# masnottuh/point-cloud-toolbox

Measured on AMD Instinct MI355X. Metric: points/sec curvature (1M-pt torus, k=50); HBM GB/s k-NN vs peak, higher is better.
Workload: dtype f64

## Files before the change

point-cloud-toolbox_amd/csrc/pct_knn.hip:

```cpp
#include "pct_knn_sweep.h"

namespace {

__global__ __launch_bounds__(256) void k_plain_records(const float* __restrict__ xyz, int64_t n, float4* __restrict__ out) {
    const int64_t i = (int64_t)blockIdx.x * 256 + threadIdx.x;
    if (i < n) out[i] = make_float4(xyz[3 * i], xyz[3 * i + 1], xyz[3 * i + 2], __int_as_float((int)i));
}

template <int R>
__global__ __launch_bounds__(64 * kWavesPerBlock) void k_query_points(const float4* __restrict__ pts, int n, const double* __restrict__ q_xyz,
                                                                      int64_t m, int k, double eps2, int* __restrict__ idx_out,
                                                                      double* __restrict__ dist_out) {
    __shared__ double s_pend_d[kWavesPerBlock][64 * R + 64];
    __shared__ int s_pend_p[kWavesPerBlock][64 * R + 64];
    const int w = __builtin_amdgcn_readfirstlane(threadIdx.x >> 6);
    const int lane = lane_id();
    const int64_t q = (int64_t)blockIdx.x * kWavesPerBlock + w;
    if (q >= m) return;
    Sweep<R> sw;
    sw.k = k - 1;
    sw.eps2 = eps2;
    sw.pts = pts;
    sw.pend_d = s_pend_d[w];
    sw.pend_p = s_pend_p[w];
// ... 175 lines not shown
    ctx->tm.sweep_variant = p.variant();
    return PCT_OK;
}

}

int pct_launch_knn_grid(pct_ctx* ctx, int32_t k, double eps, bool exact_only, int phase, bool want_dist, pct_call_clock* clock) {
    const int64_t n_rows = ctx->own_flag ? ctx->own_count : ctx->q_end - ctx->q_begin;
    const SweepPlan plan = plan_for(ctx, k, eps, false, exact_only, phase, want_dist);
    if (phase != 2) {
        PCT_TRY(reserve_table(ctx, k, eps, plan.dist));
        PCT_TRY(pct_reserve(ctx, &ctx->redo, ((size_t)n_rows + 16) * sizeof(int)));
        if (ctx->level_mode) PCT_TRY(pct_reserve(ctx, &ctx->redo_m, ((size_t)n_rows + 16) * sizeof(int)));
    }
    KnnArgs a = make_args(ctx, k, eps, true);
    if (!ctx->dist_valid) a.nbr_dist = nullptr;
    int* redo_count = &pct_dev(ctx)->sweep.redo_count;
    int* redo = (int*)ctx->redo.p;
    const dim3 block(64 * kWavesPerBlock);
    const bool fast = plan.family != kNoSweep;
    a.stamp_sweep = clock->word(PCT_ST_GRID_END);
    a.stamp_exact = clock->word(fast ? PCT_ST_FAST_END : PCT_ST_GRID_END);
    a.stamp_exact_also = fast ? nullptr : clock->word(PCT_ST_FAST_END);
    PCT_TRY(launch_sweep(ctx, plan, a, redo, redo_count));
    PCT_HIP(ctx, clock->boundary(PCT_ST_FAST_END, ctx->stream));
    if (phase != 1) {
        const int64_t waves = exact_only ? n_rows : 32768;
        const int blocks = (int)((waves + kWavesPerBlock - 1) / kWavesPerBlock);
        const int* list = exact_only ? nullptr : redo;
        if (k + 1 <= 64)
            PCT_LAUNCH(k_knn_exact<1>, dim3(blocks), block, 0, ctx->stream, a, list, (const int*)redo_count);
        else if (k + 1 <= 128)
            PCT_LAUNCH(k_knn_exact<2>, dim3(blocks), block, 0, ctx->stream, a, list, (const int*)redo_count);
        else
            PCT_TRY(pct_launch_knn_exact_wide(ctx, a, blocks, list, (const int*)redo_count));
        PCT_HIP(ctx, hipGetLastError());
    }
    ctx->knn_sorted_space = true;
    return PCT_OK;
}

int pct_launch_knn_tree(pct_ctx* ctx, int32_t k, double eps, bool want_dist, pct_call_clock* clock) {
    if (ctx->level_mode || ctx->own_flag || ctx->q_begin != 0 || ctx->q_end != ctx->n)
        return pct_fail(ctx, PCT_ERR_INVALID, "the tree sweep takes whole clouds");
    const int64_t n_rows = ctx->n;
    const bool exact_only = pct_getenv("PCT_TREE_EXACT_ONLY") != nullptr;
// ... 122 lines not shown
```

point-cloud-toolbox_amd/csrc/pct_knn_duo.hip:

```cpp
#include "pct_knn_item.h"

namespace {

#include "pct_sort_duo.inc"

__device__ __forceinline__ void sort_duo_asm(unsigned& ea, unsigned& eb, const SortLanes& c) {
    unsigned ta, tb;
    asm volatile(PCT_SORT_DUO_ASM
                 : [ea] "+v"(ea), [eb] "+v"(eb), [ta] "=&v"(ta), [tb] "=&v"(tb)
                 : [sel0] "v"(c.sel[0]), [sel1] "v"(c.sel[1]), [sel2] "v"(c.sel[2]), [sel3] "v"(c.sel[3]), [sel4] "v"(c.sel[4]),
                   [sel5] "v"(c.sel[5]), [a31] "v"(c.a31), [a63] "v"(c.a63));
    const unsigned lo = PCT_SORT_DUO_RESULT_A, hi = PCT_SORT_DUO_RESULT_B;
    ea = lo;
    eb = hi;
}

#ifndef PCT_DUO_CAP
#define PCT_DUO_CAP 768
#endif
constexpr int kDuoCap = PCT_DUO_CAP;
template <bool DIST, int CAP>
struct DuoLds {
    float cx[CAP], cy[CAP], cz[CAP];
    unsigned short pend[128 + 8];
// ... 6 lines not shown
__global__ __launch_bounds__(64, ((TREE ? PCT_TREE_CAP2 : PCT_DUO_CAP) <= 768 ? 4 : 3)) void k_knn_duo(PairArgs a) {
    constexpr int CAP = TREE ? PCT_TREE_CAP2 : kDuoCap, LIST = 128, SLOT_BITS = 7, KEY_BITS = 32 - SLOT_BITS;
    static_assert(CAP % 128 == 0 && CAP <= 1024, "slot ids: 10 bits of slot, 4 bits of run index");
    __shared__ DuoLds<DIST, CAP> L;
    const int lane = lane_id();
    const int item = a.items_per_xcd ? ((int)blockIdx.x & 7) * a.items_per_xcd + ((int)blockIdx.x >> 3) : (int)blockIdx.x;
    if (item >= a.n_items) return;
    const SortLanes sort_dir = make_sort_lanes();
    constexpr int NRUNS = TREE ? 27 : 9;
    const int2 it2 = a.items[item];
    if (item_of_split_segment<TREE>(it2)) return;
    ItemHead<TREE> head;
    load_item_head<TREE>(a, it2, lane, head);
    const int cx = head.cx, cy = head.cy, cz = head.cz, qs = head.qs, nq = head.nq, row0 = head.row0;
    const int run_s = head.run_s, run_len = head.run_len;
    const pct_grid& G = TREE ? head.g_lvl : a.g;
    float4 my_q;
    double my_qx, my_qy, my_qz;
    float my_eq;
    load_queries<Q64>(a.pts, a.ptsd, qs, nq, lane, my_q, my_qx, my_qy, my_qz, my_eq);
    int my_pre, m;
    run_prefix<NRUNS>(run_len, lane, my_pre, m);
    pct_stamp(a.stamp);
    if (item_overflows<TREE, NRUNS>(m, CAP, run_len, lane)) {
        hand_item_to_redo(a.redo, a.redo_count, a.counters, a.stats, row0, nq, lane, true);
        return;
    }
    unsigned slotx[CAP / 64];
    {
        unsigned* bits = (unsigned*)L.pend;
        static_assert(sizeof(L.pend) >= CAP / 8, "the run-start bit string lives in the survivor list");
        if (lane < CAP / 32) bits[lane] = 0u;
        wave_lds_sync();
        const bool nonempty = lane < NRUNS && run_len > 0;
        const unsigned long long ne = __builtin_amdgcn_ballot_w64(nonempty);
        if (nonempty) {
            atomicOr(&bits[my_pre >> 5], 1u << (my_pre & 31));
            L.offc[__builtin_amdgcn_mbcnt_lo((unsigned)ne, 0)] = run_s - my_pre;
        }
        wave_lds_sync();
        float4 tmp[CAP / 64];
        int ubase = -1;
#pragma unroll
        for (int b = 0; b < CAP / 64; ++b) {
            tmp[b] = make_float4(0.f, 0.f, 0.f, 0.f);
            slotx[b] = (unsigned)(b * 64 + lane);
            if (b * 64 < m) {
                const unsigned lo = (unsigned)__builtin_amdgcn_readfirstlane((int)bits[2 * b]);
                const unsigned hi = (unsigned)__builtin_amdgcn_readfirstlane((int)bits[2 * b + 1]);
                const unsigned long long B = ((unsigned long long)hi << 32) | lo;
                const unsigned long long S = B >> 1;
                const int s0 = ubase + (int)(lo & 1u);
                const int u = (int)__builtin_amdgcn_mbcnt_hi((unsigned)(S >> 32), __builtin_amdgcn_mbcnt_lo((unsigned)S, (unsigned)s0));
                ubase += (int)__popcll(B);
                const int j = b * 64 + lane;
                slotx[b] |= (unsigned)u << 10;
                if (j < m) tmp[b] = a.pts[j + L.offc[u]];
// ... 3 lines not shown
#pragma unroll
        for (int b = 0; b < CAP / 64; ++b) {
            const int j = b * 64 + lane;
            if (j < m) {
                L.cx[j] = tmp[b].x; L.cy[j] = tmp[b].y; L.cz[j] = tmp[b].z;
            } else if ((b & ~1) * 64 < m) {
                L.cx[j] = INFINITY; L.cy[j] = 0.f; L.cz[j] = 0.f;
            }
        }
    }
    wave_lds_sync();

    const int k = a.k;
    const double eps2 = EPS ? a.eps2 : (double)INFINITY;
    const KeySetup<KEY_BITS> keys = make_key_setup<KEY_BITS, EPS>(G, cx, cy, cz, my_q, Q64, my_qx, my_qy, my_qz, eps2);
    const double scale = keys.scale;
    constexpr unsigned key_max = KeySetup<KEY_BITS>::key_max;
    const unsigned my_gkey = keys.my_gkey;
    const float cell2f = keys.cell2f;
    const unsigned eps_key = EPS ? keys.eps_key : 0xFFFFFFFFu;
    const float eps2a = EPS ? keys.eps2a : INFINITY;
    const double eps1 = EPS ? keys.eps1 : 0.0;
    float t_prev_f = 0.f;
    unsigned long long redo_mask = 0ull;

    char* const pos_item = (char*)(a.nbr_pos + (int64_t)row0 * a.pitch);
    char* const dist_item = DIST ? (char*)(a.nbr_dist + (int64_t)row0 * a.pitch) : nullptr;
    const unsigned pitch4 = (unsigned)a.pitch * 4u;
    const unsigned lane_off0 = (unsigned)(lane - 1) * 4u, lane_off1 = (unsigned)(lane + 63) * 4u;
    const bool col0 = lane >= 1 && lane <= k, col1 = lane + 64 <= k;
    const unsigned long long order_lo = k >= 63 ? ~0ull : (2ull << k) - 1ull;
    const unsigned long long order_hi = k < 64 ? 0ull : k - 64 >= 63 ? ~0ull : (2ull << (k - 64)) - 1ull;
    const unsigned short* pend_hi = &L.pend[64];

    const auto query_loop = [&](auto NBP_) {
        constexpr int NBP = decltype(NBP_)::value, NBU = 2 * NBP;
        for (int qi = 0; qi < nq; ++qi) {
            const float ax = __int_as_float(__builtin_amdgcn_readlane(__float_as_int(my_q.x), qi));
            const float ay = __int_as_float(__builtin_amdgcn_readlane(__float_as_int(my_q.y), qi));
            const float az = __int_as_float(__builtin_amdgcn_readlane(__float_as_int(my_q.z), qi));
            const auto rl64 = [&](double v, int l) {
                return __hiloint2double(__builtin_amdgcn_readlane(__double2hiint(v), l), __builtin_amdgcn_readlane(__double2loint(v), l));
            };
            const double qx = Q64 ? rl64(my_qx, qi) : (double)ax, qy = Q64 ? rl64(my_qy, qi) : (double)ay, qz = Q64 ? rl64(my_qz, qi) : (double)az;
            const float eq = Q64 ? __int_as_float(__builtin_amdgcn_readlane(__float_as_int(my_eq), qi)) : 0.f;
            float ap[NBU];
#pragma unroll
// ... 22 lines not shown
            float T = T_init;
            int cnt = tot;
            unsigned bkey = 0xFFFFFFFFu;
            if (need) {
                const float target = 0.5f * (float)(k + 1 + LIST);
                float t = t_prev_f > 0.f ? t_prev_f : cell2f;
                if (!(t < T_init)) t = 0.5f * T_init;
                float lo = 0.f, hi = T_init;
                bool found = false;
#pragma unroll 1
                for (int trial = 0; trial < 16; ++trial) {
                    int c = 0;
#pragma unroll
                    for (int b = 0; b < NBU; ++b) c += (int)__popcll(__builtin_amdgcn_ballot_w64(ap[b] < t));
                    if ((unsigned)(c - (k + 1)) <= (unsigned)(LIST - (k + 1))) { T = t; cnt = c; found = true; break; }
                    const bool below = c < k + 1;
                    lo = below ? t : lo;
                    hi = below ? hi : t;
                    float nt = t * target * __builtin_amdgcn_rcpf((float)c);
                    if (!(nt > lo && nt < hi)) nt = hi < INFINITY ? 0.5f * (lo + hi) : 2.f * lo;
                    if (__builtin_amdgcn_ballot_w64(!(nt > lo && nt < hi)) != 0ull) break;
                    t = nt;
                }
                if (!found || __builtin_amdgcn_ballot_w64(!(T >= 1e-30f)) != 0ull) { redo_mask |= 1ull << qi; continue; }
                t_prev_f = T;
                double lo2 = (double)T * (1.0 - 0x1p-20);
                if constexpr (Q64) {
                    const double root_up = (double)__builtin_sqrtf(T) * (1.0 + 0x1p-21);
                    lo2 = fmax(lo2 - 2.0 * (double)eq * root_up, 0.0);
                }
                bkey = (unsigned)fmin(lo2 * scale, 4294967294.0);
            }
            {
                unsigned wr = (unsigned)(uintptr_t)&L.pend[0], wr1;
                const unsigned long long all = __builtin_amdgcn_read_exec();
                wave_lds_sync();
#pragma unroll
                for (int b = 0; b < NBU; b += 2) {
                    unsigned r0, r1, n0, n1;
                    asm volatile(
                        "v_cmp_gt_f32 vcc, %[t], %[ap0]\n"
                        "v_cmp_gt_f32 s[96:97], %[t], %[ap1]\n"
                        "s_bcnt1_i32_b64 %[n0], vcc\n"
                        "v_mbcnt_lo_u32_b32 %[r0], vcc_lo, 0\n"
                        "s_bcnt1_i32_b64 %[n1], s[96:97]\n"
                        "v_mbcnt_lo_u32_b32 %[r1], s96, 0\n"
                        "v_mbcnt_hi_u32_b32 %[r0], vcc_hi, %[r0]\n"
                        "v_mbcnt_hi_u32_b32 %[r1], s97, %[r1]\n"
                        "s_lshl1_add_u32 %[wr1], %[n0], %[wr]\n"
                        "v_lshl_add_u32 %[r0], %[r0], 1, %[wr]\n"
                        "v_lshl_add_u32 %[r1], %[r1], 1, %[wr1]\n"
                        "s_mov_b64 exec, vcc\n"
                        "ds_write_b16 %[r0], %[slot0]\n"
                        "s_mov_b64 exec, s[96:97]\n"
// ... 11 lines not shown
            unsigned e[2];
            {
                const double dx0 = (double)L.cx[j0] - qx, dy0 = (double)L.cy[j0] - qy, dz0 = (double)L.cz[j0] - qz;
                const double dx1 = (double)L.cx[j1] - qx, dy1 = (double)L.cy[j1] - qy, dz1 = (double)L.cz[j1] - qz;
                const double d20 = (dx0 * dx0 + dy0 * dy0) + dz0 * dz0;
                const double d21 = (dx1 * dx1 + dy1 * dy1) + dz1 * dz1;
                L.pay_p[lane] = j0 + L.offc[sx0 >> 10];
                L.pay_p[lane + 64] = j1 + L.offc[sx1 >> 10];
                if constexpr (DIST) {
                    L.pay_d[lane] = (float)sqrt(d20);
                    L.pay_d[lane + 64] = (float)sqrt(d21);
                }
                const unsigned k0 = (min((unsigned)(d20 * scale), key_max - 1u) << SLOT_BITS) | (unsigned)lane;
                const unsigned k1 = (min((unsigned)(d21 * scale), key_max - 1u) << SLOT_BITS) | (unsigned)(lane + 64);
                e[0] = lane < cnt && (!EPS || d20 < eps2) ? k0 : kPadElem;
                e[1] = lane + 64 < cnt && (!EPS || d21 < eps2) ? k1 : kPadElem;
            }
            wave_lds_sync();
            sort_duo_asm(e[0], e[1], sort_dir);
            const unsigned tau = (unsigned)__builtin_amdgcn_readlane((int)(k < 64 ? e[0] : e[1]), k & 63);
            const unsigned gk = (unsigned)__builtin_amdgcn_readlane((int)my_gkey, qi);
            const unsigned tk = tau >> SLOT_BITS;
            const unsigned need_k = min(tau == kPadElem ? 0xFFFFFFFFu : tk + 1u, eps_key);
            if (need_k > min(gk, bkey) || (tau != kPadElem && tk >= key_max - 1u)) { redo_mask |= 1ull << qi; continue; }
            {
                unsigned n0, n1;
                asm("s_nop 1\n"
                    "v_mov_b32_dpp %0, %2 wave_shl:1 row_mask:0xf bank_mask:0xf bound_ctrl:1\n"
                    "v_mov_b32_dpp %1, %3 wave_shl:1 row_mask:0xf bank_mask:0xf bound_ctrl:1\n"
                    "s_nop 0"
                    : "=&v"(n0), "=&v"(n1) : "v"(e[0]), "v"(e[1]));
                n0 = lane == 63 ? (unsigned)__builtin_amdgcn_readlane((int)e[1], 0) : n0;
                const bool same0 = ((e[0] ^ n0) >> SLOT_BITS) == 0u && e[0] != kPadElem && n0 != kPadElem;
                const bool same1 = ((e[1] ^ n1) >> SLOT_BITS) == 0u && e[1] != kPadElem && n1 != kPadElem && lane < 63;
                const unsigned long long cm = (__builtin_amdgcn_ballot_w64(same0) & order_lo) | (__builtin_amdgcn_ballot_w64(same1) & order_hi);
                if (__builtin_expect(cm != 0ull, 0)) {
                    const bool done = order_equal_keys<2, SLOT_BITS>(e, a.pts,
                        [&](unsigned at) {
                            const int j = min((int)L.pend[at] & 1023, CAP - 1);
                            const double dx = (double)L.cx[j] - qx, dy = (double)L.cy[j] - qy, dz = (double)L.cz[j] - qz;
                            return (dx * dx + dy * dy) + dz * dz;
                        },
                        [&](unsigned at) { return L.pay_p[at]; });
                    if (!done) { redo_mask |= 1ull << qi; continue; }
                }
            }
            {
                const unsigned off0 = lane_off0 + (unsigned)qi * pitch4, off1 = lane_off1 + (unsigned)qi * pitch4;
                const bool real0 = e[0] != kPadElem, real1 = e[1] != kPadElem;
                const int s0 = (int)(e[0] & 127u), s1 = (int)(e[1] & 127u);
                const int pos0 = L.pay_p[s0], pos1 = L.pay_p[s1];
                if (col0) *(int*)(pos_item + off0) = real0 ? pos0 : -1;
                if (col1) *(int*)(pos_item + off1) = real1 ? pos1 : -1;
                if constexpr (DIST) {
                    const float d0 = L.pay_d[s0], d1 = L.pay_d[s1];
                    if (col0) *(float*)(dist_item + off0) = real0 ? d0 : INFINITY;
                    if (col1) *(float*)(dist_item + off1) = real1 ? d1 : INFINITY;
                }
                if constexpr (EPS) {
                    const int f = (int)__popcll(__builtin_amdgcn_ballot_w64(real0 && col0)) + (int)__popcll(__builtin_amdgcn_ballot_w64(real1 && col1));
                    if (lane == 0) a.nbr_cnt[row0 + qi] = f;
                }
            }
            wave_lds_sync();
        }
    };
    {
// ... 34 lines not shown
```

point-cloud-toolbox_amd/csrc/pct_knn_fast.hip:

```cpp
#include "pct_knn_item.h"

namespace {


#ifndef PCT_FAST_WAVES
#define PCT_FAST_WAVES 4
#endif
template <int R> constexpr int kFastWaves = PCT_FAST_WAVES;



template <int R, bool EPS, bool PRE, bool PAIR = false, bool Q64 = false, bool TREE = false>
__global__ __launch_bounds__(64 * kFastWaves<R>, (TREE ? (R == 1 ? (PCT_TREE_CAP <= 512 ? 6 : PCT_TREE_CAP <= 768 ? 4 : 3) : (PCT_TREE_CAP2 <= 768 ? 4 : 3)) : R == 1 ? (Q64 ? 5 : 6) : 4)) void k_knn_fast(KnnArgs a, const int2* __restrict__ items, int64_t n_items,
                                                                  int items_q, int* __restrict__ redo,
                                                                  int* __restrict__ redo_count) {
    constexpr int CAP = TREE ? (R == 1 ? PCT_TREE_CAP : PCT_TREE_CAP2) : R == 1 ? kStageCap : PCT_STAGE_CAP2;
    constexpr int SLOT_BITS = PRE ? (R == 1 ? 6 : 7) : (R == 1 ? 9 : 10);
    constexpr int KEY_BITS = 32 - SLOT_BITS;
    constexpr int CAP_POW2 = 1024;
    static_assert(CAP <= CAP_POW2, "staging capacity");
    static_assert(PRE || CAP <= (1 << SLOT_BITS), "slot field too narrow");
    __shared__ float s_cx[kFastWaves<R>][CAP];
    __shared__ float s_cy[kFastWaves<R>][CAP];
    __shared__ float s_cz[kFastWaves<R>][CAP];
// ... 68 lines not shown
    if constexpr (Q64) {
        const double ex = my_qd.x - (double)my_q.x, ey = my_qd.y - (double)my_q.y, ez = my_qd.z - (double)my_q.z;
        my_eq = (float)sqrt((ex * ex + ey * ey) + ez * ez) * (1.0f + 0x1p-22f);
        if (!(my_eq >= 0.f)) my_eq = INFINITY;
    }
    int my_pre, m;
    run_prefix<NRUNS>(run_len, lane, my_pre, m);
    pct_stamp(a.stamp_sweep);
    unsigned long long n_flush = 0, n_step = 0, n_redo = 0;
    unsigned long long redo_mask = 0ull, redo_why_lo = 0ull, redo_why_hi = 0ull;
    const auto note_redo = [&](int row, int why) {
        const int q = row - row0;
        redo_mask |= 1ull << q;
        redo_why_lo |= (unsigned long long)(why & 1) << q;
        redo_why_hi |= (unsigned long long)((why >> 1) & 1) << q;
    };

    const bool hopeless = !EPS && a.row_done != nullptr && m < a.k + 1;
    if (item_overflows<TREE, NRUNS>(m, CAP, run_len, lane) || hopeless) {
        if (a.row_done) {
            if (lane < nq) a.redo_m[row0 + lane] = ((hopeless ? 1 : 2) << 29) | min(m, (1 << 29) - 1);
            return;
        }
        hand_item_to_redo(redo, redo_count, a.counters, a.stats, row0, nq, lane, !hopeless);
        return;
    }

    unsigned run_code[(CAP / 64 + 7) / 8];
#pragma unroll
    for (int i = 0; i < (CAP / 64 + 7) / 8; ++i) run_code[i] = 0u;
    {
        unsigned* bits = pend;
        static_assert(CAP / 32 <= 64 * R, "bit string does not fit the list area");
        if (lane < CAP / 32) bits[lane] = 0u;
        wave_lds_sync();
        const bool nonempty = lane < NRUNS && run_len > 0;
        const unsigned long long ne = __builtin_amdgcn_ballot_w64(nonempty);
        if (nonempty) {
            atomicOr(&bits[my_pre >> 5], 1u << (my_pre & 31));
            offc[__builtin_amdgcn_mbcnt_lo((unsigned)ne, 0)] = run_s - my_pre;
        }
        wave_lds_sync();
        float4 tmp[CAP / 64];
        int ubase = -1;
#pragma unroll
        for (int b = 0; b < CAP / 64; ++b) {
            tmp[b] = make_float4(0.f, 0.f, 0.f, 0.f);
// ... 686 lines not shown
```

point-cloud-toolbox_amd/csrc/pct_knn_item.h:

```cpp
#pragma once
#include "pct_knn_net.h"

namespace {

typedef float float2v __attribute__((ext_vector_type(2)));

struct PairArgs {
    const float4* pts;
    const double4* ptsd;
    const int* cell_start;
    const int* cell_own;
    const int* own_start;
    const int2* items;
    int* nbr_pos;
    float* nbr_dist;
    int* nbr_cnt;
    int* redo;
    int* redo_count;
    pct_sweep_words* counters;
    int n_items, items_q;
    int items_per_xcd;
    int k, pitch;
    int stats;
    unsigned magic_x, magic_xy;
    int shift_x, shift_xy;
    double eps2;
    pct_grid g;
    const int4* tree_seg;
    const int2* tree_runs;
    int tree_bits;
    unsigned long long* stamp;
};

PairArgs make_pair_args(const pct_ctx* ctx, const KnnArgs& a, bool tree, int* redo, int* redo_count) {
    PairArgs pa = {};
    pa.pts = a.pts; pa.ptsd = a.ptsd; pa.cell_start = a.cell_start;
    pa.items = (const int2*)ctx->occ.p;
    pa.nbr_pos = a.nbr_pos; pa.nbr_dist = a.nbr_dist; pa.nbr_cnt = a.nbr_cnt;
    pa.redo = redo; pa.redo_count = redo_count; pa.counters = a.counters;
    pa.n_items = (int)ctx->n_items; pa.items_q = ctx->items_q;
    pa.k = a.k; pa.pitch = a.pitch; pa.stats = a.stats; pa.eps2 = a.eps2; pa.g = a.g;
    pa.stamp = a.stamp_sweep;
    pa.items_per_xcd = pct_getenv("PCT_NO_XCD_MAP") ? 0 : (int)((ctx->n_items + 7) / 8);
    if (tree) {
        pa.tree_seg = a.tree_seg; pa.tree_runs = a.tree_runs; pa.tree_bits = a.tree_bits;
        return pa;
    }
    pa.cell_own = a.cell_own; pa.own_start = a.own_start;
    const auto magic = [](unsigned d, unsigned* mg, int* sh) {
        int l = 0;
        while ((1ull << l) < d) ++l;
        *sh = 30 + l;
        *mg = (unsigned)(((1ull << *sh) + d - 1) / d);
    };
    magic((unsigned)a.g.nx, &pa.magic_x, &pa.shift_x);
    magic((unsigned)a.g.nx * (unsigned)a.g.ny, &pa.magic_xy, &pa.shift_xy);
    return pa;
}

template <class F, class... Rest>
void with_bools(F&& f, bool b, Rest... rest) {
    if constexpr (sizeof...(rest) == 0) {
        if (b) f(std::true_type{}); else f(std::false_type{});
    } else {
// ... 74 lines not shown
        }
    }
}

template <int NRUNS>
__device__ __forceinline__ void run_prefix(const int run_len, const int lane, int& my_pre, int& m) {
    my_pre = 0;
    int acc = 0;
#pragma unroll
    for (int t = 0; t < NRUNS; ++t) {
        my_pre = lane == t ? acc : my_pre;
        acc += __builtin_amdgcn_readlane(run_len, t);
    }
    m = acc;
}

template <bool TREE, int NRUNS>
__device__ __forceinline__ bool item_overflows(const int m, const int cap, const int run_len, const int lane) {
    const bool crowded = TREE && __popcll(__builtin_amdgcn_ballot_w64(lane < NRUNS && run_len > 0)) > 16;
    return m > cap || crowded;
}

__device__ __forceinline__ void hand_item_to_redo(int* __restrict__ redo, int* __restrict__ redo_count, pct_sweep_words* counters,
                                                  const int stats, const int row0, const int nq, const int lane, const bool overflow) {
    int base = 0;
    if (lane == 0) base = atomicAdd(redo_count, nq);
    base = __builtin_amdgcn_readfirstlane(base);
    if (lane < nq) redo[base + lane] = row0 + lane;
    if (stats && lane == 0) {
        if (overflow) atomicAdd(&counters->lds_overflows, 1ull);
        atomicAdd(&counters->redone_queries, (unsigned long long)nq);
    }
}

template <bool Q64>
__device__ __forceinline__ void load_queries(const float4* pts, const double4* ptsd, const int qs, const int nq,
                                             const int lane, float4& my_q, double& my_qx, double& my_qy, double& my_qz, float& my_eq) {
    my_q = make_float4(0.f, 0.f, 0.f, 0.f);
    my_qx = 0.; my_qy = 0.; my_qz = 0.;
    my_eq = 0.f;
    if (lane < nq) {
        my_q = pts[qs + lane];
        if constexpr (Q64) {
            const double4 qd = ptsd[qs + lane];
            my_qx = qd.x; my_qy = qd.y; my_qz = qd.z;
        }
    }
    if constexpr (Q64) {
        const double ex = my_qx - (double)my_q.x, ey = my_qy - (double)my_q.y, ez = my_qz - (double)my_q.z;
        my_eq = (float)sqrt((ex * ex + ey * ey) + ez * ez) * (1.0f + 0x1p-22f);
        if (!(my_eq >= 0.f)) my_eq = INFINITY;
// ... 38 lines not shown
```

point-cloud-toolbox_amd/csrc/pct_knn_pair.hip:

```cpp
#include "pct_knn_item.h"

namespace {

#ifndef PCT_SORT_INC
#define PCT_SORT_INC "pct_sort_pair.inc"
#endif
#include PCT_SORT_INC

__device__ __forceinline__ void sort_pair_asm(unsigned& ea, unsigned& eb, const SortLanes& c) {
    unsigned ta, tb;
    asm volatile(PCT_SORT_PAIR_ASM
                 : [ea] "+v"(ea), [eb] "+v"(eb), [ta] "=&v"(ta), [tb] "=&v"(tb)
                 : [sel0] "v"(c.sel[0]), [sel1] "v"(c.sel[1]), [sel2] "v"(c.sel[2]), [sel3] "v"(c.sel[3]), [sel4] "v"(c.sel[4]),
                   [sel5] "v"(c.sel[5]), [a31] "v"(c.a31), [a63] "v"(c.a63));
    ea = PCT_SORT_PAIR_RESULT_A;
    eb = PCT_SORT_PAIR_RESULT_B;
}

constexpr int kPairCap = kStageCap;
static_assert((kPairCap & (kPairCap - 1)) == 0 && kPairCap % 128 == 0 && kPairCap <= 512, "staging capacity of k_knn_pair");
static_assert(PCT_TREE_CAP % 128 == 0 && PCT_TREE_CAP <= 1024, "staging capacity of k_knn_pair on the hierarchical cell list");
template <int CAP>
struct PairLdsT {
    float cx[CAP], cy[CAP], cz[CAP];
// ... 16 lines not shown
    __shared__ PairLdsT<CAP> s_lds[kPairWaves];
    const int w = kPairWaves == 1 ? 0 : __builtin_amdgcn_readfirstlane(threadIdx.x >> 6);
    const int lane = lane_id();
    const int blk = (int)blockIdx.x * kPairWaves + w;
    const int item = a.items_per_xcd ? (blk & 7) * a.items_per_xcd + (blk >> 3) : blk;
    if (item >= a.n_items || (a.items_per_xcd && (blk >> 3) >= a.items_per_xcd)) return;
    PairLdsT<CAP>& L = s_lds[w];
    const SortLanes sort_dir = make_sort_lanes();
    constexpr int NRUNS = TREE ? 27 : 9;
    const int2 it2 = a.items[item];
    if (item_of_split_segment<TREE>(it2)) return;
    ItemHead<TREE> head;
    load_item_head<TREE>(a, it2, lane, head);
    const int cx = head.cx, cy = head.cy, cz = head.cz, qs = head.qs, nq = head.nq, row0 = head.row0;
    const int run_s = head.run_s, run_len = head.run_len;
    const pct_grid& G = TREE ? head.g_lvl : a.g;
    float4 my_q;
    double my_qx, my_qy, my_qz;
    float my_eq;
    load_queries<Q64>(a.pts, a.ptsd, qs, nq, lane, my_q, my_qx, my_qy, my_qz, my_eq);
    int my_pre, m;
    run_prefix<NRUNS>(run_len, lane, my_pre, m);
    pct_stamp(a.stamp);
    if (item_overflows<TREE, NRUNS>(m, CAP, run_len, lane)) {
        hand_item_to_redo(a.redo, a.redo_count, a.counters, a.stats, row0, nq, lane, true);
        return;
    }

    unsigned slotx[CAP / 64];
    {
        unsigned* bits = L.pend;
        if (lane < CAP / 32) bits[lane] = 0u;
        wave_lds_sync();
        const bool nonempty = lane < NRUNS && run_len > 0;
        const unsigned long long ne = __builtin_amdgcn_ballot_w64(nonempty);
        if (nonempty) {
            atomicOr(&bits[my_pre >> 5], 1u << (my_pre & 31));
            L.offc[__builtin_amdgcn_mbcnt_lo((unsigned)ne, 0)] = run_s - my_pre;
        }
        wave_lds_sync();
        float4 tmp[CAP / 64];
        int ubase = -1;
#pragma unroll
        for (int b = 0; b < CAP / 64; ++b) {
            tmp[b] = make_float4(0.f, 0.f, 0.f, 0.f);
            slotx[b] = (unsigned)(b * 64 + lane);
            if (b * 64 < m) {
                const unsigned lo = (unsigned)__builtin_amdgcn_readfirstlane((int)bits[2 * b]);
                const unsigned hi = (unsigned)__builtin_amdgcn_readfirstlane((int)bits[2 * b + 1]);
                const unsigned long long B = ((unsigned long long)hi << 32) | lo;
                const unsigned long long S = B >> 1;
                const int s0 = ubase + (int)(lo & 1u);
                const int u = (int)__builtin_amdgcn_mbcnt_hi((unsigned)(S >> 32), __builtin_amdgcn_mbcnt_lo((unsigned)S, (unsigned)s0));
                ubase += (int)__popcll(B);
                const int j = b * 64 + lane;
                slotx[b] |= (unsigned)u << SB;
                if (j < m) tmp[b] = a.pts[j + L.offc[u]];
// ... 3 lines not shown
#pragma unroll
        for (int b = 0; b < CAP / 64; ++b) {
            const int j = b * 64 + lane;
            if (j < m) {
                L.cx[j] = tmp[b].x; L.cy[j] = tmp[b].y; L.cz[j] = tmp[b].z;
            } else if ((b & ~1) * 64 < m) {
                L.cx[j] = INFINITY; L.cy[j] = 0.f; L.cz[j] = 0.f;
            }
        }
    }
    wave_lds_sync();

    const int k = a.k;
    const double eps2 = EPS ? a.eps2 : (double)INFINITY;
    const KeySetup<KEY_BITS> keys = make_key_setup<KEY_BITS, EPS>(G, cx, cy, cz, my_q, Q64, my_qx, my_qy, my_qz, eps2);
    const double scale = keys.scale;
    constexpr unsigned key_max = KeySetup<KEY_BITS>::key_max;
    const unsigned my_gkey = keys.my_gkey;
    const float cell2f = keys.cell2f;
    const unsigned eps_key = EPS ? keys.eps_key : 0xFFFFFFFFu;
    const float eps2a = EPS ? keys.eps2a : INFINITY;
    const double eps1 = EPS ? keys.eps1 : 0.0;
    float t_prev_f = 0.f;
    unsigned long long redo_mask = 0ull;

    char* const pos_item = (char*)(a.nbr_pos + (int64_t)row0 * a.pitch);
    char* const dist_item = DIST ? (char*)(a.nbr_dist + (int64_t)row0 * a.pitch) : nullptr;
    const unsigned lane_off = (unsigned)(lane - 1) * 4u;
    const unsigned pitch4 = (unsigned)a.pitch * 4u;
    const bool col_lane = lane >= 1 && lane <= k;
    const unsigned long long first_k1 = (2ull << k) - 1ull;

    static_assert(CAP <= (1 << SB) && SB + 4 <= 16, "slot ids: SB bits of slot, 4 bits of run index, 16-bit survivor list of query b");
    const auto slot_of = [](unsigned id) { return TREE ? min((int)(id & ((1u << SB) - 1u)), CAP - 1) : (int)(id & (unsigned)(CAP - 1)); };

    const auto pair_loop = [&](auto NBP_) {
        constexpr int NBP = decltype(NBP_)::value, NBU = 2 * NBP;
        for (int qi = 0; qi < nq; qi += 2) {
            const bool live_b = qi + 1 < nq;
            const int qj = live_b ? qi + 1 : qi;
            const float ax = __int_as_float(__builtin_amdgcn_readlane(__float_as_int(my_q.x), qi));
            const float ay = __int_as_float(__builtin_amdgcn_readlane(__float_as_int(my_q.y), qi));
            const float az = __int_as_float(__builtin_amdgcn_readlane(__float_as_int(my_q.z), qi));
            const float bx = __int_as_float(__builtin_amdgcn_readlane(__float_as_int(my_q.x), qj));
            const float by = __int_as_float(__builtin_amdgcn_readlane(__float_as_int(my_q.y), qj));
            const float bz = __int_as_float(__builtin_amdgcn_readlane(__float_as_int(my_q.z), qj));
            const auto rl64 = [&](double v, int l) {
// ... 83 lines not shown
                    float nt = v_t * target * __builtin_amdgcn_rcpf((float)c);
                    if (!(nt > v_lo && nt < v_hi)) nt = v_hi < INFINITY ? 0.5f * (v_lo + v_hi) : 2.f * v_lo;
                    go = go && nt > v_lo && nt < v_hi;
                    v_t = go ? nt : v_t;
                    if ((__builtin_amdgcn_ballot_w64(go) & 3ull) == 0ull) break;
                }
                const unsigned fm = (unsigned)__builtin_amdgcn_ballot_w64(found);
                T_a = __int_as_float(__builtin_amdgcn_readlane(__float_as_int(v_T), 0));
                T_b = __int_as_float(__builtin_amdgcn_readlane(__float_as_int(v_T), 1));
                cnt_a = __builtin_amdgcn_readlane(v_cnt, 0);
                cnt_b = __builtin_amdgcn_readlane(v_cnt, 1);
                double lo2 = (double)v_T * (1.0 - 0x1p-20);
                if constexpr (Q64) {
                    const double root_up = (double)__builtin_sqrtf(v_T) * (1.0 + 0x1p-21);
                    lo2 = fmax(lo2 - 2.0 * (double)v_eq * root_up, 0.0);
                }
                const unsigned v_bkey = (unsigned)fmin(lo2 * scale, 4294967294.0);
                ok_a = (fm & 1u) != 0u && (!need_a || T_a >= 1e-30f);
                ok_b = live_b && (fm & 2u) != 0u && (!need_b || T_b >= 1e-30f);
                if (need_a && ok_a) { t_prev_f = T_a; bkey_a = (unsigned)__builtin_amdgcn_readlane((int)v_bkey, 0); }
                if (need_b && ok_b) { t_prev_f = T_b; bkey_b = (unsigned)__builtin_amdgcn_readlane((int)v_bkey, 1); }
                if (!ok_a) { redo_mask |= 1ull << qi; T_a = 0.f; cnt_a = 0; }
                if (!ok_b) { if (live_b) redo_mask |= 1ull << qj; T_b = 0.f; cnt_b = 0; }
                if (!ok_a && !ok_b) continue;
            }
            if (!live_b) { T_b = 0.f; cnt_b = 0; }
            {
                unsigned wr_a = (unsigned)(uintptr_t)&L.pend[0], wr_b = (unsigned)(uintptr_t)&L.pend_b[0];
                const unsigned long long all = __builtin_amdgcn_read_exec();
                wave_lds_sync();
#ifndef PCT_ABL_NO_COMPACT
#pragma unroll
                for (int b = 0; b < NBU; ++b) {
                    unsigned ra, rb, ca, cb;
                    const unsigned slot = slotx[b];
                    asm volatile(
                        "v_cmp_gt_f32 vcc, %[ta], %[apa]\n"
                        "v_cmp_gt_f32 s[96:97], %[tb], %[apb]\n"
                        "s_bcnt1_i32_b64 %[ca], vcc\n"
                        "v_mbcnt_lo_u32_b32 %[ra], vcc_lo, 0\n"
                        "s_bcnt1_i32_b64 %[cb], s[96:97]\n"
                        "v_mbcnt_lo_u32_b32 %[rb], s96, 0\n"
                        "v_mbcnt_hi_u32_b32 %[ra], vcc_hi, %[ra]\n"
                        "v_mbcnt_hi_u32_b32 %[rb], s97, %[rb]\n"
                        "v_lshl_add_u32 %[ra], %[ra], 2, %[wra]\n"
                        "v_lshl_add_u32 %[rb], %[rb], 1, %[wrb]\n"
                        "s_mov_b64 exec, vcc\n"
// ... 84 lines not shown
                            [&](unsigned at) {
                                const int j = slot_of((unsigned)L.pend_b[at]);
                                const double dx = (double)L.cx[j] - ux, dy = (double)L.cy[j] - uy, dz = (double)L.cz[j] - uz;
                                return (dx * dx + dy * dy) + dz * dz;
                            },
                            [&](unsigned at) { return __builtin_amdgcn_ds_bpermute((int)(at & 63u) << 2, out_pb); });
                        if (!done) { redo_mask |= 1ull << qj; ok_b = false; }
                    }
                }
            }
            {
                const unsigned off_a = lane_off + (unsigned)qi * pitch4, off_b = lane_off + (unsigned)qj * pitch4;
                const bool real_a = e_a != kPadElem, real_b = e_b != kPadElem;
                const int at_a = (int)(e_a << 2), at_b = (int)(e_b << 2);
                const int pos_a = __builtin_amdgcn_ds_bpermute(at_a, out_pa), pos_b = __builtin_amdgcn_ds_bpermute(at_b, out_pb);
                float dist_a = 0.f, dist_b = 0.f;
                if constexpr (DIST) {
                    dist_a = __int_as_float(__builtin_amdgcn_ds_bpermute(at_a, __float_as_int(out_da)));
                    dist_b = __int_as_float(__builtin_amdgcn_ds_bpermute(at_b, __float_as_int(out_db)));
                }
#ifdef PCT_ABL_NO_STORE
                if (pos_a == 0x7fffffff && pos_b == 0x7ffffff1)
#endif
                if (ok_a && col_lane) {
                    *(int*)(pos_item + off_a) = real_a ? pos_a : -1;
                    if constexpr (DIST) *(float*)(dist_item + off_a) = real_a ? dist_a : INFINITY;
                }
#ifdef PCT_ABL_NO_STORE
                if (pos_a == 0x7fffffff && pos_b == 0x7ffffff1)
#endif
                if (ok_b && col_lane) {
                    *(int*)(pos_item + off_b) = real_b ? pos_b : -1;
                    if constexpr (DIST) *(float*)(dist_item + off_b) = real_b ? dist_b : INFINITY;
                }
                if constexpr (EPS) {
                    const int f_a = (int)__popcll(__builtin_amdgcn_ballot_w64(real_a && col_lane));
                    const int f_b = (int)__popcll(__builtin_amdgcn_ballot_w64(real_b && col_lane));
                    if (lane == 0) {
                        if (ok_a) a.nbr_cnt[row0 + qi] = f_a;
                        if (ok_b) a.nbr_cnt[row0 + qj] = f_b;
                    }
                }
            }
        }
    };
    {
        using std::integral_constant;
        const int nbp = (m + 127) >> 7;
        if (nbp <= 1) pair_loop(integral_constant<int, 1>{});
        else if (nbp == 2) pair_loop(integral_constant<int, 2>{});
        else if (nbp == 3) pair_loop(integral_constant<int, (CAP >= 384 ? 3 : 1)>{});
        else if (nbp == 4) pair_loop(integral_constant<int, (CAP >= 512 ? 4 : 1)>{});
        else if (nbp == 5) pair_loop(integral_constant<int, (CAP >= 640 ? 5 : 1)>{});
        else pair_loop(integral_constant<int, (CAP >= 768 ? 6 : 1)>{});
// ... 28 lines not shown
```

point-cloud-toolbox_amd/csrc/pct_knn_sweep.h:

```cpp
#pragma once
#include "pct_internal.h"
#include "pct_query_plan.h"
#include "pct_sweep_plan.h"

#include <math.h>
#include <type_traits>

struct KnnArgs {
    const float4* pts;
    const double4* ptsd;
    const int* cell_start;
    const int* cell_own;
    const int* own_start;
    const int* owned_pos;
    int64_t n_owned;
    const int* occ;
    int64_t n_occ;
    int64_t n;
    pct_grid g;
    int k;
    int pitch;
    double eps2;
    int q_begin, q_end;
    int* nbr_pos;
    float* nbr_dist;
    int* nbr_cnt;
    int* row_done;
    int* redo_m;
    const int4* tree_seg;
    const int2* tree_runs;
    int tree_bits;
    const unsigned long long* tree_codes;
    const unsigned char* tree_lvl;
    const int* tree_bucket;
    int stats;
    pct_sweep_words* counters;
    unsigned long long* stamp_sweep;
    unsigned long long* stamp_exact;
    unsigned long long* stamp_exact_also;
};

int pct_launch_knn_exact_wide(pct_ctx* ctx, const KnnArgs& a, int blocks, const int* list, const int* list_count);
int pct_launch_knn_brute_wide(pct_ctx* ctx, const KnnArgs& a, int blocks);
void pct_launch_sweep_fast(pct_ctx* ctx, const SweepPlan& p, const KnnArgs& a, int* redo, int* redo_count);
void pct_launch_sweep_pair(pct_ctx* ctx, const SweepPlan& p, const KnnArgs& a, int* redo, int* redo_count);
void pct_launch_sweep_duo(pct_ctx* ctx, const SweepPlan& p, const KnnArgs& a, int* redo, int* redo_count);

namespace {

constexpr int kWavesPerBlock = 4;
constexpr int kStageCap = PCT_STAGE_CAP;
constexpr int PCT_STAGE_CAP2_HOST = PCT_STAGE_CAP2;


__device__ __forceinline__ int lane_id() { return threadIdx.x & 63; }

__device__ __forceinline__ void wave_lds_sync() {
    __builtin_amdgcn_fence(__ATOMIC_RELEASE, "wavefront");
    __builtin_amdgcn_wave_barrier();
    __builtin_amdgcn_fence(__ATOMIC_ACQUIRE, "wavefront");
}

// ... 109 lines not shown
    const float4* pts;
    double* pend_d;
    int* pend_p;

    __device__ __forceinline__ void reset() {
#pragma unroll
        for (int r = 0; r < R; ++r) {
            best.d[r] = INFINITY;
            best.p[r] = INT_MAX;
        }
        tau_d = INFINITY;
        tau_p = INT_MAX;
        npend = 0;
        empty = true;
    }

    __device__ __forceinline__ void refresh_tau() {
        const int slot = k >> 6, src = k & 63;
        double d = best.d[0];
        int p = best.p[0];
#pragma unroll
        for (int r = 1; r < R; ++r)
            if (slot == r) { d = best.d[r]; p = best.p[r]; }
        tau_d = __shfl(d, src);
        tau_p = __shfl(p, src);
    }

    __device__ __forceinline__ void flush() {
        const int lane = lane_id();
        TopK<R> b;
        wave_lds_sync();
        const int take = npend < 64 * R ? npend : 64 * R;
#pragma unroll
        for (int r = 0; r < R; ++r) {
            const int i = lane + 64 * r;
            const bool v = i < take;
            b.d[r] = v ? pend_d[i] : INFINITY;
            b.p[r] = v ? pend_p[i] : INT_MAX;
        }
        const int rest = npend - take;
        double md = 0;
        int mp = 0;
        if (lane < rest) { md = pend_d[take + lane]; mp = pend_p[take + lane]; }
        wave_lds_sync();
        if (lane < rest) { pend_d[lane] = md; pend_p[lane] = mp; }
        wave_lds_sync();
        npend = rest;
        bitonic_sort_from<R, 2>(b, !empty, pts);
        if (empty) {
            best = b;
            empty = false;
        } else {
            bitonic_merge_min<R>(best, b, pts);
        }
        refresh_tau();
    }

    __device__ __forceinline__ void consider(float4 c, int pos, bool valid) {
        const double dx = (double)c.x - qx, dy = (double)c.y - qy, dz = (double)c.z - qz;
        const double d2 = (dx * dx + dy * dy) + dz * dz;
        const bool closer = key_less(d2, valid ? pos : INT_MAX, tau_d, tau_p, pts);
        const bool pass = valid && d2 < eps2 && closer;
        const unsigned long long m = __ballot(pass);
        if (pass) {
            const int slot = npend + __builtin_amdgcn_mbcnt_hi((unsigned)(m >> 32), __builtin_amdgcn_mbcnt_lo((unsigned)m, 0));
            pend_d[slot] = d2;
            pend_p[slot] = pos;
        }
        npend += __popcll(m);
    }

    __device__ __forceinline__ void store(int64_t row, int pitch, int* nbr_pos, float* nbr_dist, int* nbr_cnt) {
        const int lane = lane_id();
        int found = 0;
#pragma unroll
        for (int r = 0; r < R; ++r) {
            const int i = lane + 64 * r;
            const bool real = best.p[r] != INT_MAX;
            if (i >= 1 && i <= k) {
                nbr_pos[row * pitch + (i - 1)] = real ? best.p[r] : -1;
                if (nbr_dist) nbr_dist[row * pitch + (i - 1)] = real ? (float)sqrt(best.d[r]) : INFINITY;
                found += real;
            }
        }
        if (nbr_cnt) {
// ... 122 lines not shown
    sw.k = a.k;
    sw.eps2 = a.eps2;
    sw.pts = a.pts;
    sw.pend_d = s_pend_d[w];
    sw.pend_p = s_pend_p[w];

    for (int64_t item = (int64_t)blockIdx.x * kWavesPerBlock + w; item < total; item += nwaves) {
        const int row = list ? list[item] : (int)item;
        const int q = a.owned_pos[row];
        const float4 qp = a.pts[q];
        const int cx = __builtin_amdgcn_readfirstlane(cell_coord_d((double)qp.x, g.ox, g.inv_cell, g.nx));
        const int cy = __builtin_amdgcn_readfirstlane(cell_coord_d((double)qp.y, g.oy, g.inv_cell, g.ny));
        const int cz = __builtin_amdgcn_readfirstlane(cell_coord_d((double)qp.z, g.oz, g.inv_cell, g.nz));
        if (a.ptsd) {
            const double4 qd = a.ptsd[q];
            sw.qx = qd.x; sw.qy = qd.y; sw.qz = qd.z;
        } else {
            sw.qx = (double)qp.x; sw.qy = (double)qp.y; sw.qz = (double)qp.z;
        }
        sw.reset();
        const double gx = (sw.qx - g.ox) * g.inv_cell - cx;
        const double gy = (sw.qy - g.oy) * g.inv_cell - cy;
        const double gz = (sw.qz - g.oz) * g.inv_cell - cz;
        ShellIter it;
        it.start(g, cy, cz, -1, 1);
        int nbase = 0, nlim = 0;
        bool have_next = it.next(g, cs, cx, cy, cz, nbase, nlim);
        float4 c_next = make_float4(0.f, 0.f, 0.f, 0.f);
        if (have_next && nbase + lane < nlim) c_next = a.pts[nbase + lane];
        for (;;) {
            const bool have = have_next;
            if (have) {
                const int pos = nbase + lane;
                const bool valid = pos < nlim;
                const float4 c = c_next;
                have_next = it.next(g, cs, cx, cy, cz, nbase, nlim);
                if (have_next && nbase + lane < nlim) c_next = a.pts[nbase + lane];
                sw.consider(c, pos, valid);
                if (sw.npend < 64 * R) continue;
            }
            if (sw.npend > 0 || sw.empty) sw.flush();
            if (have) continue;
            if (fmin(sw.tau_d, sw.eps2) <= guaranteed_r2(g, cx, cy, cz, gx, gy, gz, it.ring)) {
                if (lane == 0 && fmin(sw.tau_d, sw.eps2) > limit_r2(g, cx, cy, cz, gx, gy, gz)) atomicAdd(&a.counters->beyond_limits, 1ull);
                break;
            }
            it.start(g, cy, cz, it.ring, it.ring < 4 ? it.ring + 1 : it.ring + (it.ring + 1) / 2, fmin(sw.tau_d, sw.eps2), gx, gy, gz);
            have_next = it.next(g, cs, cx, cy, cz, nbase, nlim);
// ... 131 lines not shown
```

Measured before the change: 1.539 billion.

## Seed exact k-NN redo pass with partial neighbor lists from the fast sweep

```diff
diff --git a/point-cloud-toolbox_amd/csrc/pct_knn.hip b/point-cloud-toolbox_amd/csrc/pct_knn.hip
--- a/point-cloud-toolbox_amd/csrc/pct_knn.hip
+++ b/point-cloud-toolbox_amd/csrc/pct_knn.hip
@@ -221,6 +221,8 @@
     a.stamp_sweep = clock->word(PCT_ST_GRID_END);
     a.stamp_exact = clock->word(fast ? PCT_ST_FAST_END : PCT_ST_GRID_END);
     a.stamp_exact_also = fast ? nullptr : clock->word(PCT_ST_FAST_END);
+    const char* seed_env = pct_getenv("PCT_REDO_SEED");
+    a.redo_seed = plan.lean() && !plan.tree && phase == 0 && !(seed_env && seed_env[0] == '0' && seed_env[1] == 0);
     PCT_TRY(launch_sweep(ctx, plan, a, redo, redo_count));
     PCT_HIP(ctx, clock->boundary(PCT_ST_FAST_END, ctx->stream));
     if (phase != 1) {
diff --git a/point-cloud-toolbox_amd/csrc/pct_knn_duo.hip b/point-cloud-toolbox_amd/csrc/pct_knn_duo.hip
--- a/point-cloud-toolbox_amd/csrc/pct_knn_duo.hip
+++ b/point-cloud-toolbox_amd/csrc/pct_knn_duo.hip
@@ -52,9 +52,15 @@
     int my_pre, m;
     run_prefix<NRUNS>(run_len, lane, my_pre, m);
     pct_stamp(a.stamp);
+    unsigned long long redo_mask = 0ull;
     if (item_overflows<TREE, NRUNS>(m, CAP, run_len, lane)) {
-        hand_item_to_redo(a.redo, a.redo_count, a.counters, a.stats, row0, nq, lane, true);
-        return;
+        if (TREE || !a.seed) {
+            hand_item_to_redo(a.redo, a.redo_count, a.counters, a.stats, row0, nq, lane, true, a.nbr_pos, a.pitch);
+            return;
+        }
+        redo_mask = nq >= 64 ? ~0ull : (1ull << nq) - 1ull;
+        if (a.stats && lane == 0) atomicAdd(&a.counters->lds_overflows, 1ull);
+        m = CAP;
     }
     unsigned slotx[CAP / 64];
     {
@@ -62,7 +68,7 @@
         static_assert(sizeof(L.pend) >= CAP / 8, "the run-start bit string lives in the survivor list");
         if (lane < CAP / 32) bits[lane] = 0u;
         wave_lds_sync();
-        const bool nonempty = lane < NRUNS && run_len > 0;
+        const bool nonempty = lane < NRUNS && run_len > 0 && my_pre < CAP;
         const unsigned long long ne = __builtin_amdgcn_ballot_w64(nonempty);
         if (nonempty) {
             atomicOr(&bits[my_pre >> 5], 1u << (my_pre & 31));
@@ -112,7 +118,6 @@
     const float eps2a = EPS ? keys.eps2a : INFINITY;
     const double eps1 = EPS ? keys.eps1 : 0.0;
     float t_prev_f = 0.f;
-    unsigned long long redo_mask = 0ull;
 
     char* const pos_item = (char*)(a.nbr_pos + (int64_t)row0 * a.pitch);
     char* const dist_item = DIST ? (char*)(a.nbr_dist + (int64_t)row0 * a.pitch) : nullptr;
@@ -181,14 +186,19 @@
                     if (__builtin_amdgcn_ballot_w64(!(nt > lo && nt < hi)) != 0ull) break;
                     t = nt;
                 }
-                if (!found || __builtin_amdgcn_ballot_w64(!(T >= 1e-30f)) != 0ull) { redo_mask |= 1ull << qi; continue; }
-                t_prev_f = T;
-                double lo2 = (double)T * (1.0 - 0x1p-20);
-                if constexpr (Q64) {
-                    const double root_up = (double)__builtin_sqrtf(T) * (1.0 + 0x1p-21);
-                    lo2 = fmax(lo2 - 2.0 * (double)eq * root_up, 0.0);
-                }
-                bkey = (unsigned)fmin(lo2 * scale, 4294967294.0);
+                if (!found || __builtin_amdgcn_ballot_w64(!(T >= 1e-30f)) != 0ull) {
+                    redo_mask |= 1ull << qi;
+                    T = 0.f;
+                    cnt = 0;
+                } else {
+                    t_prev_f = T;
+                    double lo2 = (double)T * (1.0 - 0x1p-20);
+                    if constexpr (Q64) {
+                        const double root_up = (double)__builtin_sqrtf(T) * (1.0 + 0x1p-21);
+                        lo2 = fmax(lo2 - 2.0 * (double)eq * root_up, 0.0);
+                    }
+                    bkey = (unsigned)fmin(lo2 * scale, 4294967294.0);
+                }
             }
             {
                 unsigned wr = (unsigned)(uintptr_t)&L.pend[0], wr1;
@@ -246,7 +256,7 @@
             const unsigned gk = (unsigned)__builtin_amdgcn_readlane((int)my_gkey, qi);
             const unsigned tk = tau >> SLOT_BITS;
             const unsigned need_k = min(tau == kPadElem ? 0xFFFFFFFFu : tk + 1u, eps_key);
-            if (need_k > min(gk, bkey) || (tau != kPadElem && tk >= key_max - 1u)) { redo_mask |= 1ull << qi; continue; }
+            if (need_k > min(gk, bkey) || (tau != kPadElem && tk >= key_max - 1u)) redo_mask |= 1ull << qi;
             {
                 unsigned n0, n1;
                 asm("s_nop 1\n"
@@ -258,7 +268,7 @@
                 const bool same0 = ((e[0] ^ n0) >> SLOT_BITS) == 0u && e[0] != kPadElem && n0 != kPadElem;
                 const bool same1 = ((e[1] ^ n1) >> SLOT_BITS) == 0u && e[1] != kPadElem && n1 != kPadElem && lane < 63;
                 const unsigned long long cm = (__builtin_amdgcn_ballot_w64(same0) & order_lo) | (__builtin_amdgcn_ballot_w64(same1) & order_hi);
-                if (__builtin_expect(cm != 0ull, 0)) {
+                if (__builtin_expect(cm != 0ull && ((redo_mask >> qi) & 1ull) == 0ull, 0)) {
                     const bool done = order_equal_keys<2, SLOT_BITS>(e, a.pts,
                         [&](unsigned at) {
                             const int j = min((int)L.pend[at] & 1023, CAP - 1);
@@ -266,7 +276,7 @@
                             return (dx * dx + dy * dy) + dz * dz;
                         },
                         [&](unsigned at) { return L.pay_p[at]; });
-                    if (!done) { redo_mask |= 1ull << qi; continue; }
+                    if (!done) redo_mask |= 1ull << qi;
                 }
             }
             {
diff --git a/point-cloud-toolbox_amd/csrc/pct_knn_fast.hip b/point-cloud-toolbox_amd/csrc/pct_knn_fast.hip
--- a/point-cloud-toolbox_amd/csrc/pct_knn_fast.hip
+++ b/point-cloud-toolbox_amd/csrc/pct_knn_fast.hip
@@ -114,7 +114,7 @@
             if (lane < nq) a.redo_m[row0 + lane] = ((hopeless ? 1 : 2) << 29) | min(m, (1 << 29) - 1);
             return;
         }
-        hand_item_to_redo(redo, redo_count, a.counters, a.stats, row0, nq, lane, !hopeless);
+        hand_item_to_redo(redo, redo_count, a.counters, a.stats, row0, nq, lane, !hopeless, a.nbr_pos, a.pitch);
         return;
     }
 
diff --git a/point-cloud-toolbox_amd/csrc/pct_knn_item.h b/point-cloud-toolbox_amd/csrc/pct_knn_item.h
--- a/point-cloud-toolbox_amd/csrc/pct_knn_item.h
+++ b/point-cloud-toolbox_amd/csrc/pct_knn_item.h
@@ -22,6 +22,7 @@
     int items_per_xcd;
     int k, pitch;
     int stats;
+    int seed;
     unsigned magic_x, magic_xy;
     int shift_x, shift_xy;
     double eps2;
@@ -40,6 +41,7 @@
     pa.redo = redo; pa.redo_count = redo_count; pa.counters = a.counters;
     pa.n_items = (int)ctx->n_items; pa.items_q = ctx->items_q;
     pa.k = a.k; pa.pitch = a.pitch; pa.stats = a.stats; pa.eps2 = a.eps2; pa.g = a.g;
+    pa.seed = a.redo_seed;
     pa.stamp = a.stamp_sweep;
     pa.items_per_xcd = pct_getenv("PCT_NO_XCD_MAP") ? 0 : (int)((ctx->n_items + 7) / 8);
     if (tree) {
@@ -160,11 +162,15 @@
 }
 
 __device__ __forceinline__ void hand_item_to_redo(int* __restrict__ redo, int* __restrict__ redo_count, pct_sweep_words* counters,
-                                                  const int stats, const int row0, const int nq, const int lane, const bool overflow) {
+                                                  const int stats, const int row0, const int nq, const int lane, const bool overflow,
+                                                  int* __restrict__ nbr_pos, const int pitch) {
     int base = 0;
     if (lane == 0) base = atomicAdd(redo_count, nq);
     base = __builtin_amdgcn_readfirstlane(base);
-    if (lane < nq) redo[base + lane] = row0 + lane;
+    if (lane < nq) {
+        redo[base + lane] = row0 + lane;
+        nbr_pos[(int64_t)(row0 + lane) * pitch] = -1;
+    }
     if (stats && lane == 0) {
         if (overflow) atomicAdd(&counters->lds_overflows, 1ull);
         atomicAdd(&counters->redone_queries, (unsigned long long)nq);
diff --git a/point-cloud-toolbox_amd/csrc/pct_knn_pair.hip b/point-cloud-toolbox_amd/csrc/pct_knn_pair.hip
--- a/point-cloud-toolbox_amd/csrc/pct_knn_pair.hip
+++ b/point-cloud-toolbox_amd/csrc/pct_knn_pair.hip
@@ -62,9 +62,15 @@
     int my_pre, m;
     run_prefix<NRUNS>(run_len, lane, my_pre, m);
     pct_stamp(a.stamp);
+    unsigned long long redo_mask = 0ull;
     if (item_overflows<TREE, NRUNS>(m, CAP, run_len, lane)) {
-        hand_item_to_redo(a.redo, a.redo_count, a.counters, a.stats, row0, nq, lane, true);
-        return;
+        if (TREE || !a.seed) {
+            hand_item_to_redo(a.redo, a.redo_count, a.counters, a.stats, row0, nq, lane, true, a.nbr_pos, a.pitch);
+            return;
+        }
+        redo_mask = nq >= 64 ? ~0ull : (1ull << nq) - 1ull;
+        if (a.stats && lane == 0) atomicAdd(&a.counters->lds_overflows, 1ull);
+        m = CAP;
     }
 
     unsigned slotx[CAP / 64];
@@ -72,7 +78,7 @@
         unsigned* bits = L.pend;
         if (lane < CAP / 32) bits[lane] = 0u;
         wave_lds_sync();
-        const bool nonempty = lane < NRUNS && run_len > 0;
+        const bool nonempty = lane < NRUNS && run_len > 0 && my_pre < CAP;
         const unsigned long long ne = __builtin_amdgcn_ballot_w64(nonempty);
         if (nonempty) {
             atomicOr(&bits[my_pre >> 5], 1u << (my_pre & 31));
@@ -122,7 +128,6 @@
     const float eps2a = EPS ? keys.eps2a : INFINITY;
     const double eps1 = EPS ? keys.eps1 : 0.0;
     float t_prev_f = 0.f;
-    unsigned long long redo_mask = 0ull;
 
     char* const pos_item = (char*)(a.nbr_pos + (int64_t)row0 * a.pitch);
     char* const dist_item = DIST ? (char*)(a.nbr_dist + (int64_t)row0 * a.pitch) : nullptr;
@@ -252,7 +257,6 @@
                 if (need_b && ok_b) { t_prev_f = T_b; bkey_b = (unsigned)__builtin_amdgcn_readlane((int)v_bkey, 1); }
                 if (!ok_a) { redo_mask |= 1ull << qi; T_a = 0.f; cnt_a = 0; }
                 if (!ok_b) { if (live_b) redo_mask |= 1ull << qj; T_b = 0.f; cnt_b = 0; }
-                if (!ok_a && !ok_b) continue;
             }
             if (!live_b) { T_b = 0.f; cnt_b = 0; }
             {
@@ -383,14 +387,14 @@
 #ifdef PCT_ABL_NO_STORE
                 if (pos_a == 0x7fffffff && pos_b == 0x7ffffff1)
 #endif
-                if (ok_a && col_lane) {
+                if (col_lane) {
                     *(int*)(pos_item + off_a) = real_a ? pos_a : -1;
                     if constexpr (DIST) *(float*)(dist_item + off_a) = real_a ? dist_a : INFINITY;
                 }
 #ifdef PCT_ABL_NO_STORE
                 if (pos_a == 0x7fffffff && pos_b == 0x7ffffff1)
 #endif
-                if (ok_b && col_lane) {
+                if (live_b && col_lane) {
                     *(int*)(pos_item + off_b) = real_b ? pos_b : -1;
                     if constexpr (DIST) *(float*)(dist_item + off_b) = real_b ? dist_b : INFINITY;
                 }
diff --git a/point-cloud-toolbox_amd/csrc/pct_knn_sweep.h b/point-cloud-toolbox_amd/csrc/pct_knn_sweep.h
--- a/point-cloud-toolbox_amd/csrc/pct_knn_sweep.h
+++ b/point-cloud-toolbox_amd/csrc/pct_knn_sweep.h
@@ -38,6 +38,7 @@
     unsigned long long* stamp_sweep;
     unsigned long long* stamp_exact;
     unsigned long long* stamp_exact_also;
+    int redo_seed;
 };
 
 int pct_launch_knn_exact_wide(pct_ctx* ctx, const KnnArgs& a, int blocks, const int* list, const int* list_count);
@@ -193,8 +194,52 @@
 #pragma unroll
         for (int r = 1; r < R; ++r)
             if (slot == r) { d = best.d[r]; p = best.p[r]; }
-        tau_d = __shfl(d, src);
-        tau_p = __shfl(p, src);
+        d = __shfl(d, src);
+        p = __shfl(p, src);
+        if (p != INT_MAX) { tau_d = d; tau_p = p; }
+    }
+
+    __device__ __forceinline__ double dist2(const float4 c) const {
+        const double dx = (double)c.x - qx, dy = (double)c.y - qy, dz = (double)c.z - qz;
+        return (dx * dx + dy * dy) + dz * dz;
+    }
+
+    __device__ __forceinline__ double seed(const int* __restrict__ cols, const int self, const int n) {
+        const int lane = lane_id();
+        int p[R];
+        bool bad = false;
+        double B = dist2(pts[self]);
+#pragma unroll
+        for (int r = 0; r < R; ++r) {
+            const int col = lane + 64 * r;
+            p[r] = col < k ? cols[col] : -1;
+            if (col < k) {
+                const bool in = (unsigned)p[r] < (unsigned)n && p[r] != self;
+                bad = bad || !in;
+                const double d2 = dist2(pts[in ? p[r] : self]);
+                bad = bad || !(d2 < INFINITY);
+                B = fmax(B, d2);
+            }
+        }
+        if (__ballot(bad) != 0ull) return INFINITY;
+        for (int i = 0; i + 1 < k; ++i) {
+            int v = p[0];
+#pragma unroll
+            for (int r = 1; r < R; ++r)
+                if ((i >> 6) == r) v = p[r];
+            v = __builtin_amdgcn_readlane(v, i & 63);
+#pragma unroll
+            for (int r = 0; r < R; ++r) {
+                const int col = lane + 64 * r;
+                bad = bad || (col > i && col < k && p[r] == v);
+            }
+        }
+        if (__ballot(bad) != 0ull) return INFINITY;
+        for (int o = 32; o > 0; o >>= 1) B = fmax(B, __shfl_xor(B, o));
+        if (!(B < INFINITY)) return INFINITY;
+        tau_d = B;
+        tau_p = INT_MAX;
+        return B;
     }
 
     __device__ __forceinline__ void flush() {
@@ -228,10 +273,10 @@
     }
 
     __device__ __forceinline__ void consider(float4 c, int pos, bool valid) {
-        const double dx = (double)c.x - qx, dy = (double)c.y - qy, dz = (double)c.z - qz;
-        const double d2 = (dx * dx + dy * dy) + dz * dz;
+        const double d2 = dist2(c);
         const bool closer = key_less(d2, valid ? pos : INT_MAX, tau_d, tau_p, pts);
-        const bool pass = valid && d2 < eps2 && closer;
+        const bool at_seed = tau_p == INT_MAX && d2 == tau_d && d2 < INFINITY;
+        const bool pass = valid && d2 < eps2 && (closer || at_seed);
         const unsigned long long m = __ballot(pass);
         if (pass) {
             const int slot = npend + __builtin_amdgcn_mbcnt_hi((unsigned)(m >> 32), __builtin_amdgcn_mbcnt_lo((unsigned)m, 0));
@@ -400,8 +445,9 @@
         const double gx = (sw.qx - g.ox) * g.inv_cell - cx;
         const double gy = (sw.qy - g.oy) * g.inv_cell - cy;
         const double gz = (sw.qz - g.oz) * g.inv_cell - cz;
+        const double seed_d2 = a.redo_seed && list ? sw.seed(a.nbr_pos + (int64_t)row * a.pitch, q, (int)a.n) : (double)INFINITY;
         ShellIter it;
-        it.start(g, cy, cz, -1, 1);
+        it.start(g, cy, cz, -1, 1, seed_d2, gx, gy, gz);
         int nbase = 0, nlim = 0;
         bool have_next = it.next(g, cs, cx, cy, cz, nbase, nlim);
         float4 c_next = make_float4(0.f, 0.f, 0.f, 0.f);
```

Measured after the change: 1.561 billion, median of 6. 1.01x the previous value.
